# NVIDIA-Merlin/NVTabular

Hardware: AMD Instinct MI355X
Metric: rows/sec + GB/s (Criteo Categorify+FillMissing+Normalize fit+transform, HBM-resident) (higher is better)
Workload: dtype int32 keys -> int64 labels; fp64 moments/normalize; 1 GPU; synthetic Criteo-day0: 26 int32 categorical (Criteo-1TB cardinalities, Zipf) + 13 int32 continuous, nulls as Arrow bitmaps; Categorify + FillMissing + Normalize, fit + transform; rows_per_gpu=45000000, algorithmic_bytes_per_row=624, tie_break=value (count desc, value asc), artifacts=deferred (no parquet I/O inside the timed region)

## Files before the change

### nvtabular_amd/csrc/nvt_sort.hip

```cpp
#include <type_traits>

#include <cstdlib>

#include "nvt_common.hpp"
#include "nvt_internal.hpp"
#include "nvt_prof.hpp"
#include "nvt_scan.hpp"
#include "nvt_sort_tile.hpp"

namespace nvt {

template <typename K>
__device__ __forceinline__ unsigned sort_digit(K key, int64_t cnt, int pass) {
  constexpr int KB = (int)sizeof(K);
  if (pass < KB) {
    using U = typename std::make_unsigned<K>::type;
    U u = (U)key ^ ((U)1 << (8 * KB - 1));
    return (unsigned)((u >> (8 * pass)) & 0xFF);
  }
  uint64_t inv = ~(uint64_t)cnt;
  return (unsigned)((inv >> (8 * (pass - KB))) & 0xFF);
}

constexpr int kSmallMax = 8192;
constexpr int kSmallBS = 1024;

template <typename K>
__device__ __forceinline__ bool vocab_before(int64_t ca, K ka, int64_t cb, K kb) {
  return ca > cb || (ca == cb && ka < kb);
}

template <typename K>
__global__ __launch_bounds__(kSmallBS) void sort_small_kernel(K *keys, int64_t *counts, unsigned n) {
  __shared__ K sk[kSmallMax];
  __shared__ int64_t sc[kSmallMax];
  unsigned m = 1;
  while (m < n) m <<= 1;
  for (unsigned i = threadIdx.x; i < m; i += kSmallBS) {
    if (i < n) {
      sk[i] = keys[i];
      sc[i] = counts[i];
    } else {
      sk[i] = std::numeric_limits<K>::max();
      sc[i] = INT64_MIN;
    }
  }
  __syncthreads();
  for (unsigned size = 2; size <= m; size <<= 1) {
    for (unsigned stride = size >> 1; stride > 0; stride >>= 1) {
      for (unsigned t = threadIdx.x; t < m / 2; t += kSmallBS) {
        unsigned lo = 2 * t - (t & (stride - 1));
        unsigned hi = lo + stride;
        bool up = (lo & size) == 0;
        K ka = sk[lo], kb = sk[hi];
        int64_t ca = sc[lo], cb = sc[hi];
        bool swap = up ? vocab_before<K>(cb, kb, ca, ka) : vocab_before<K>(ca, ka, cb, kb);
        if (swap) {
          sk[lo] = kb;
          sk[hi] = ka;
          sc[lo] = cb;
          sc[hi] = ca;
        }
      }
      __syncthreads();
    }
  }
  for (unsigned i = threadIdx.x; i < n; i += kSmallBS) {
    keys[i] = sk[i];
    counts[i] = sc[i];
  }
}

constexpr int kRows = 8;
constexpr int kTileSort = kBlock * kRows;

template <typename K>
__global__ __launch_bounds__(kBlock) void sort_pass_hist_kernel(const K *__restrict__ keys,
                                                                const int64_t *__restrict__ cnts,
                                                                uint64_t n,
                                                                unsigned long long *pass_hist) {
  constexpr int NP = (int)sizeof(K) + 8;
  __shared__ unsigned h[NP * 256];
  for (int i = threadIdx.x; i < NP * 256; i += kBlock) h[i] = 0;
  __syncthreads();
  const uint64_t stride = (uint64_t)gridDim.x * kBlock;
  for (uint64_t i = (uint64_t)blockIdx.x * kBlock + threadIdx.x; i < n; i += stride) {
    K k = keys[i];
    int64_t c = cnts[i];
#pragma unroll
    for (int p = 0; p < NP; ++p) atomicAdd(&h[p * 256 + sort_digit<K>(k, c, p)], 1u);
  }
  __syncthreads();
  for (int i = threadIdx.x; i < NP * 256; i += kBlock)
    if (h[i]) atomicAdd(&pass_hist[i], (unsigned long long)h[i]);
}

__device__ __forceinline__ uint64_t tile_elem(uint64_t tile, unsigned w, unsigned r, unsigned l) {
  return tile * kTileSort + (uint64_t)w * (kRows * kWave) + (uint64_t)r * kWave + l;
}

template <typename K>
__global__ __launch_bounds__(kBlock) void sort_tile_hist_kernel(const K *__restrict__ keys,
                                                                const int64_t *__restrict__ cnts,
                                                                uint64_t n, int pass,
                                                                unsigned *tile_hist,
                                                                uint64_t ntiles) {
  constexpr int KB = (int)sizeof(K);
  __shared__ unsigned h[256];
  h[threadIdx.x] = 0;
  __syncthreads();
  const unsigned w = threadIdx.x / kWave, l = lane_id();
#pragma unroll
  for (int r = 0; r < kRows; ++r) {
    uint64_t i = tile_elem(blockIdx.x, w, r, l);
    if (i < n) {
      unsigned d = pass < KB ? sort_digit<K>(keys[i], 0, pass) : sort_digit<K>((K)0, cnts[i], pass);
      atomicAdd(&h[d], 1u);
    }
  }
  __syncthreads();
  tile_hist[(uint64_t)threadIdx.x * ntiles + blockIdx.x] = h[threadIdx.x];
}

template <typename K>
__global__ __launch_bounds__(kBlock) void sort_scatter_kernel(
    const K *__restrict__ keys, const int64_t *__restrict__ cnts, uint64_t n, int pass,
    const unsigned *__restrict__ tile_off, uint64_t ntiles, K *out_keys, int64_t *out_cnts) {
  __shared__ unsigned wcnt[kBlock / kWave][256];
  const unsigned w = threadIdx.x / kWave, l = lane_id();
  for (int i = threadIdx.x; i < (kBlock / kWave) * 256; i += kBlock) (&wcnt[0][0])[i] = 0;
  __syncthreads();
  K k[kRows];
  int64_t c[kRows];
  unsigned dig[kRows], local[kRows];
  bool act[kRows];
#pragma unroll
  for (int r = 0; r < kRows; ++r) {
    uint64_t i = tile_elem(blockIdx.x, w, r, l);
    act[r] = i < n;
    k[r] = act[r] ? keys[i] : (K)0;
    c[r] = act[r] ? cnts[i] : 0;
    dig[r] = sort_digit<K>(k[r], c[r], pass);
  }
#pragma unroll
  for (int r = 0; r < kRows; ++r) {
    unsigned long long peers = match_digit(dig[r], act[r]);
    unsigned rank = __popcll(peers & ((1ull << l) - 1ull));
    unsigned before = act[r] ? wcnt[w][dig[r]] : 0;
    __builtin_amdgcn_wave_barrier();
    if (act[r] && rank == 0) wcnt[w][dig[r]] = before + (unsigned)__popcll(peers);
    __builtin_amdgcn_wave_barrier();
    local[r] = before + rank;
  }
  __syncthreads();
  {
    const unsigned d = threadIdx.x;
    unsigned run = tile_off[(uint64_t)d * ntiles + blockIdx.x];
#pragma unroll
    for (int q = 0; q < kBlock / kWave; ++q) {
      unsigned t = wcnt[q][d];
      wcnt[q][d] = run;
      run += t;
    }
  }
  __syncthreads();
#pragma unroll
  for (int r = 0; r < kRows; ++r) {
    if (act[r]) {
      unsigned dst = wcnt[w][dig[r]] + local[r];
      out_keys[dst] = k[r];
      out_cnts[dst] = c[r];
    }
  }
}


template <bool FIRST>
__global__ __launch_bounds__(kS2BS) void sort2_hist_kernel(const uint64_t *__restrict__ comp,
                                                           const int32_t *__restrict__ keys,
                                                           const int64_t *__restrict__ cnts,
                                                           uint64_t n, int shift,
                                                           unsigned *tile_hist, uint64_t ntiles) {
  __shared__ unsigned h[256];
  h[threadIdx.x] = 0;
  __syncthreads();
  const uint64_t base = (uint64_t)blockIdx.x * kS2Tile;
#pragma unroll 4
  for (int r = 0; r < kS2Rows; ++r) {
    const uint64_t i = base + (uint64_t)r * kS2BS + threadIdx.x;
    const bool act = i < n;
    uint64_t c = 0;
    if (act) c = FIRST ? comp_make(keys[i], cnts[i]) : comp[i];
    const unsigned d = (unsigned)(c >> shift) & 0xFF;
    if (shift < 32) {
      if (act) atomicAdd(&h[d], 1u);
    } else {
      const unsigned long long peers = match_digit(d, act);
      if (act && (peers & ((1ull << lane_id()) - 1ull)) == 0)
        atomicAdd(&h[d], (unsigned)__popcll(peers));
    }
  }
  __syncthreads();
  tile_hist[(uint64_t)threadIdx.x * ntiles + blockIdx.x] = h[threadIdx.x];
}

template <bool FIRST, bool LAST>
__global__ __launch_bounds__(kS2BS) void sort2_scatter_kernel(
    const uint64_t *__restrict__ comp, const int32_t *__restrict__ keys,
    const int64_t *__restrict__ cnts, uint64_t n, int shift, const unsigned *__restrict__ tile_off,
    const unsigned long long *__restrict__ chunk_base, uint64_t ntiles, uint64_t *out_comp,
    int32_t *out_keys, int64_t *out_cnts) {
  constexpr int NW = kS2BS / kWave;
  __shared__ unsigned wcnt[NW][256];
  __shared__ unsigned goff[256];
  __shared__ unsigned wtot[NW];
  __shared__ uint64_t stage[kS2Tile];
  const unsigned w = threadIdx.x / kWave, l = lane_id();
#pragma unroll
  for (int q = 0; q < NW; ++q) wcnt[q][threadIdx.x] = 0;
  __syncthreads();
  uint64_t c[kS2Rows];
  unsigned short local[kS2Rows];
#pragma unroll
  for (int r = 0; r < kS2Rows; ++r) {
    const uint64_t i = s2_elem(blockIdx.x, w, r, l);
    c[r] = ~0ull;
    if (i < n) c[r] = FIRST ? comp_make(keys[i], cnts[i]) : comp[i];
  }
  const uint64_t tile_base = (uint64_t)blockIdx.x * kS2Tile;
#pragma unroll
  for (int r = 0; r < kS2Rows; ++r) {
    const bool act = s2_elem(blockIdx.x, w, r, l) < n;
    const unsigned d = (unsigned)(c[r] >> shift) & 0xFF;
    const unsigned long long peers = match_digit(d, act);
    const unsigned rank = __popcll(peers & ((1ull << l) - 1ull));
    const unsigned before = act ? wcnt[w][d] : 0;
    __builtin_amdgcn_wave_barrier();
    if (act && rank == 0) wcnt[w][d] = before + (unsigned)__popcll(peers);
    __builtin_amdgcn_wave_barrier();
    local[r] = (unsigned short)(before + rank);
  }
  __syncthreads();
  {
    const unsigned d = threadIdx.x;
    unsigned t[NW], tot = 0;
#pragma unroll
    for (int q = 0; q < NW; ++q) {
      t[q] = wcnt[q][d];
      tot += t[q];
    }
    unsigned inc = tot;
#pragma unroll
    for (int off = 1; off < 64; off <<= 1) {
      unsigned o = __shfl_up(inc, off, 64);
      if (l >= (unsigned)off) inc += o;
    }
    if (l == 63) wtot[w] = inc;
    __syncthreads();
    unsigned wbase = 0;
    for (unsigned q = 0; q < w; ++q) wbase += wtot[q];
    const unsigned dstart = wbase + inc - tot;
    unsigned run = dstart;
#pragma unroll
    for (int q = 0; q < NW; ++q) {
      wcnt[q][d] = run;
      run += t[q];
    }
    goff[d] = scan_lookup(tile_off, chunk_base, (uint64_t)d * ntiles + blockIdx.x) - dstart;
  }
  __syncthreads();
#pragma unroll
  for (int r = 0; r < kS2Rows; ++r) {
    if (s2_elem(blockIdx.x, w, r, l) < n) {
      const unsigned d = (unsigned)(c[r] >> shift) & 0xFF;
      stage[wcnt[w][d] + local[r]] = c[r];
    }
  }
  __syncthreads();
  const unsigned tile_n = (unsigned)(n - tile_base < (uint64_t)kS2Tile ? n - tile_base : kS2Tile);
#pragma unroll 4
  for (int j = 0; j < kS2Rows; ++j) {
    const unsigned idx = j * kS2BS + threadIdx.x;
    if (idx < tile_n) {
      const uint64_t v = stage[idx];
      const unsigned d = (unsigned)(v >> shift) & 0xFF;
      const unsigned dst = goff[d] + idx;
      if (LAST) {
        out_keys[dst] = comp_key(v);
        out_cnts[dst] = comp_cnt(v);
      } else {
        out_comp[dst] = v;
      }
    }
  }
}

constexpr int kOsMaxPass = 8;
constexpr int kOsHistBlocks = 1024;

__global__ __launch_bounds__(kS2BS) void os_hist_kernel(const int32_t *__restrict__ keys,
                                                        const int64_t *__restrict__ cnts,
                                                        uint64_t n, int npass,
                                                        unsigned *__restrict__ block_hist) {
  __shared__ unsigned h[kOsMaxPass * 256];
  for (int i = threadIdx.x; i < npass * 256; i += kS2BS) h[i] = 0;
  __syncthreads();
  const unsigned l = lane_id();
  unsigned c255[kOsMaxPass];
#pragma unroll
  for (int p = 0; p < kOsMaxPass; ++p) c255[p] = 0;
  const uint64_t stride = (uint64_t)gridDim.x * kS2BS;
  const uint64_t iters = (n + stride - 1) / stride;
  for (uint64_t it = 0; it < iters; ++it) {
    const uint64_t i = it * stride + (uint64_t)blockIdx.x * kS2BS + threadIdx.x;
    const bool act = i < n;
    const uint64_t c = act ? comp_make(keys[i], cnts[i]) : 0ull;
#pragma unroll
    for (int p = 0; p < 4; ++p)
      if (act) atomicAdd(&h[p * 256 + ((unsigned)(c >> (8 * p)) & 0xFF)], 1u);
    if (npass > 4) {
      const unsigned d = (unsigned)(c >> 32) & 0xFF;
      const unsigned long long peers = match_digit(d, act);
      if (act && (peers & ((1ull << l) - 1ull)) == 0)
        atomicAdd(&h[4 * 256 + d], (unsigned)__popcll(peers));
    }
#pragma unroll
    for (int p = 5; p < kOsMaxPass; ++p) {
      if (p < npass && act) {
        const unsigned d = (unsigned)(c >> (8 * p)) & 0xFF;
        if (d == 0xFF)
          ++c255[p];
        else
          atomicAdd(&h[p * 256 + d], 1u);
      }
    }
  }
#pragma unroll
  for (int p = 5; p < kOsMaxPass; ++p) {
    if (p < npass) {
      unsigned v = c255[p];
#pragma unroll
      for (int off = 32; off > 0; off >>= 1) v += __shfl_down(v, off, 64);
      if (l == 0 && v) atomicAdd(&h[p * 256 + 0xFF], v);
    }
  }
  __syncthreads();
  for (int i = threadIdx.x; i < npass * 256; i += kS2BS)
    block_hist[(uint64_t)blockIdx.x * (kOsMaxPass * 256) + i] = h[i];
}

__global__ __launch_bounds__(256) void os_base_kernel(const unsigned *__restrict__ block_hist,
                                                      int nblocks, unsigned *__restrict__ base) {
  __shared__ unsigned wtot[4];
  const int p = blockIdx.x, d = threadIdx.x;
  unsigned tot = 0;
#pragma unroll 8
  for (int b = 0; b < nblocks; ++b) tot += block_hist[(uint64_t)b * (kOsMaxPass * 256) + p * 256 + d];
  unsigned inc = tot;
#pragma unroll
  for (int off = 1; off < 64; off <<= 1) {
    unsigned o = __shfl_up(inc, off, 64);
    if (lane_id() >= (unsigned)off) inc += o;
  }
  const unsigned w = threadIdx.x / kWave;
  if (lane_id() == 63) wtot[w] = inc;
  __syncthreads();
  unsigned wb = 0;
  for (unsigned q = 0; q < w; ++q) wb += wtot[q];
  base[p * 256 + d] = wb + inc - tot;
}

template <bool LAST, typename LOAD>
__device__ __forceinline__ void os_scatter_body(
    LOAD load, uint64_t n, int shift, const unsigned *__restrict__ base,
    unsigned *status, unsigned *ticket, uint64_t *out_comp, int32_t *out_keys, int64_t *out_cnts) {
  constexpr int NW = kS2BS / kWave;
  __shared__ unsigned wcnt[NW][256];
  __shared__ unsigned goff[256];
  __shared__ unsigned wtot[NW];
  __shared__ unsigned s_tile;
  __shared__ uint64_t stage[kS2Tile];
  const unsigned w = threadIdx.x / kWave, l = lane_id();
  if (threadIdx.x == 0) s_tile = atomicAdd(ticket, 1u);
#pragma unroll
  for (int q = 0; q < NW; ++q) wcnt[q][threadIdx.x] = 0;
  __syncthreads();
  const unsigned tile = s_tile;
  uint64_t c[kS2Rows];
  unsigned short local[kS2Rows];
#pragma unroll
  for (int r = 0; r < kS2Rows; ++r) {
    const uint64_t i = s2_elem(tile, w, r, l);
    c[r] = ~0ull;
    if (i < n) c[r] = load(i);
  }
  const uint64_t tile_base = (uint64_t)tile * kS2Tile;
#pragma unroll
  for (int r = 0; r < kS2Rows; ++r) {
    const bool act = s2_elem(tile, w, r, l) < n;
    const unsigned d = (unsigned)(c[r] >> shift) & 0xFF;
    const unsigned long long peers = match_digit(d, act);
    const unsigned rank = __popcll(peers & ((1ull << l) - 1ull));
    const unsigned before = act ? wcnt[w][d] : 0;
    __builtin_amdgcn_wave_barrier();
    if (act && rank == 0) wcnt[w][d] = before + (unsigned)__popcll(peers);
    __builtin_amdgcn_wave_barrier();
    local[r] = (unsigned short)(before + rank);
  }
  __syncthreads();
  {
    const unsigned d = threadIdx.x;
    unsigned t[NW], tot = 0;
#pragma unroll
    for (int q = 0; q < NW; ++q) {
      t[q] = wcnt[q][d];
      tot += t[q];
    }
    unsigned *my = status + (uint64_t)tile * 256 + d;
    __hip_atomic_store(my, (tile == 0 ? kOsPrefix : kOsAgg) | tot, __ATOMIC_RELAXED,
                       __HIP_MEMORY_SCOPE_AGENT);
    unsigned inc = tot;
#pragma unroll
    for (int off = 1; off < 64; off <<= 1) {
      unsigned o = __shfl_up(inc, off, 64);
      if (l >= (unsigned)off) inc += o;
    }
    if (l == 63) wtot[w] = inc;
    __syncthreads();
    unsigned wbase = 0;
    for (unsigned q = 0; q < w; ++q) wbase += wtot[q];
    const unsigned dstart = wbase + inc - tot;
    unsigned run = dstart;
#pragma unroll
    for (int q = 0; q < NW; ++q) {
      wcnt[q][d] = run;
      run += t[q];
    }
    unsigned excl = 0;
    if (tile > 0) {
      unsigned tb = tile - 1;
      while (true) {
        const unsigned v = __hip_atomic_load(status + (uint64_t)tb * 256 + d, __ATOMIC_RELAXED,
                                             __HIP_MEMORY_SCOPE_AGENT);
        const unsigned f = v >> 30;
        if (f == 0) {
          __builtin_amdgcn_s_sleep(1);
          continue;
        }
        excl += v & kOsMask;
        if (f == 2) break;
        --tb;
      }
      __hip_atomic_store(my, kOsPrefix | (excl + tot), __ATOMIC_RELAXED, __HIP_MEMORY_SCOPE_AGENT);
    }
    goff[d] = base[d] + excl - dstart;
  }
  __syncthreads();
#pragma unroll
  for (int r = 0; r < kS2Rows; ++r) {
    if (s2_elem(tile, w, r, l) < n) {
      const unsigned d = (unsigned)(c[r] >> shift) & 0xFF;
      stage[wcnt[w][d] + local[r]] = c[r];
    }
  }
  __syncthreads();
  const unsigned tile_n = (unsigned)(n - tile_base < (uint64_t)kS2Tile ? n - tile_base : kS2Tile);
#pragma unroll 4
  for (int j = 0; j < kS2Rows; ++j) {
    const unsigned idx = j * kS2BS + threadIdx.x;
    if (idx < tile_n) {
      const uint64_t v = stage[idx];
      const unsigned d = (unsigned)(v >> shift) & 0xFF;
      const unsigned dst = goff[d] + idx;
      if (LAST) {
        out_keys[dst] = comp_key(v);
        out_cnts[dst] = comp_cnt(v);
      } else {
        out_comp[dst] = v;
      }
    }
  }
}

template <bool FIRST, bool LAST>
__global__ __launch_bounds__(kS2BS) void os_scatter_kernel(
    const uint64_t *__restrict__ comp, const int32_t *__restrict__ keys,
    const int64_t *__restrict__ cnts, uint64_t n, int shift, const unsigned *__restrict__ base,
    unsigned *status, unsigned *ticket, uint64_t *out_comp, int32_t *out_keys, int64_t *out_cnts) {
  os_scatter_body<LAST>([=](uint64_t i) -> uint64_t { return FIRST ? comp_make(keys[i], cnts[i]) : comp[i]; },
                        n, shift, base, status, ticket, out_comp, out_keys, out_cnts);
}

template <typename K>
struct PackedKeyWord {
  const K *keys;
  const uint8_t *fold;
  int64_t bias;
  int rb;
  __device__ __forceinline__ uint64_t operator()(uint64_t i) const {
    const uint64_t img = (uint32_t)((uint64_t)(int64_t)keys[i] - (uint64_t)bias);
    const uint64_t f = fold ? (uint64_t)fold[i] : 0ull;
    return (img << 32) | (f << rb) | i;
  }
};
template <typename K>
__global__ __launch_bounds__(kS2BS) void os_scatter_pack_kernel(
    PackedKeyWord<K> src, uint64_t n, int shift, const unsigned *__restrict__ base, unsigned *status,
    unsigned *ticket, uint64_t *out_comp) {
  os_scatter_body<false>(src, n, shift, base, status, ticket, out_comp, nullptr, nullptr);
}

inline uint64_t os_tmp_bytes(uint64_t n) {
  const uint64_t ntiles = (n + kS2Tile - 1) / kS2Tile;
  return 2 * n * 8 + (uint64_t)kOsHistBlocks * kOsMaxPass * 256 * 4 + kOsMaxPass * 256 * 4 +
         (uint64_t)kOsMaxPass * ntiles * 256 * 4 + kOsMaxPass * 4 + 256;
}

inline int vocab_sort_onesweep(int32_t *keys, int64_t *counts, uint64_t n, int64_t max_count,
                               void *tmp, hipStream_t stream) {
  const uint64_t ntiles = (n + kS2Tile - 1) / kS2Tile;
  char *p = reinterpret_cast<char *>(tmp);
  uint64_t *bufs[2];
  bufs[0] = reinterpret_cast<uint64_t *>(p);
  p += n * 8;
  bufs[1] = reinterpret_cast<uint64_t *>(p);
  p += n * 8;
  unsigned *block_hist = reinterpret_cast<unsigned *>(p);
  p += (uint64_t)kOsHistBlocks * kOsMaxPass * 256 * 4;
  unsigned *base = reinterpret_cast<unsigned *>(p);
  p += kOsMaxPass * 256 * 4;
  unsigned *status = reinterpret_cast<unsigned *>(p);
  int count_bytes = 0;
  for (uint64_t m = (uint64_t)max_count; m; m >>= 8) ++count_bytes;
  const int npass = 4 + count_bytes;
  const uint64_t status_words = (uint64_t)npass * ntiles * 256;
  unsigned *tickets = status + status_words;
  NVT_CHECK_HIP(hipMemsetAsync(status, 0, (status_words + kOsMaxPass) * 4, stream));
  const unsigned hb = (unsigned)(ntiles < (uint64_t)kOsHistBlocks ? ntiles : kOsHistBlocks);
  os_hist_kernel<<<hb, kS2BS, 0, stream>>>(keys, counts, n, npass, block_hist);
  NVT_CHECK_LAUNCH();
  os_base_kernel<<<npass, 256, 0, stream>>>(block_hist, (int)hb, base);
  NVT_CHECK_LAUNCH();
  const uint64_t *src = nullptr;
  int flip = 0;
  for (int pass = 0; pass < npass; ++pass) {
    const int shift = 8 * pass;
    const bool first = pass == 0, last = pass == npass - 1;
    unsigned *st = status + (uint64_t)pass * ntiles * 256;
    uint64_t *dst = bufs[flip];
    if (first)
      os_scatter_kernel<true, false><<<(unsigned)ntiles, kS2BS, 0, stream>>>(
          nullptr, keys, counts, n, shift, base + pass * 256, st, tickets + pass, dst, nullptr,
          nullptr);
    else if (last)
      os_scatter_kernel<false, true><<<(unsigned)ntiles, kS2BS, 0, stream>>>(
          src, nullptr, nullptr, n, shift, base + pass * 256, st, tickets + pass, nullptr, keys,
          counts);
    else
      os_scatter_kernel<false, false><<<(unsigned)ntiles, kS2BS, 0, stream>>>(
          src, nullptr, nullptr, n, shift, base + pass * 256, st, tickets + pass, dst, nullptr,
          nullptr);
    NVT_CHECK_LAUNCH();
    src = dst;
    flip ^= 1;
  }
  return NVT_OK;
}

template <typename LOAD>
__device__ __forceinline__ void os_hist_words_body(LOAD load, uint64_t n, int bit_lo, int npass,
                                                   unsigned *__restrict__ block_hist) {
  __shared__ unsigned h[kOsMaxPass * 256];
  for (int i = threadIdx.x; i < npass * 256; i += kS2BS) h[i] = 0;
  __syncthreads();
  const unsigned l = lane_id();
  const uint64_t stride = (uint64_t)gridDim.x * kS2BS;
  const uint64_t iters = (n + stride - 1) / stride;
  constexpr int U = 4;
  for (uint64_t it = 0; it < iters; it += U) {
    uint64_t cw[U];
    bool av[U];
#pragma unroll
    for (int u = 0; u < U; ++u) {
      const uint64_t i = (it + u) * stride + (uint64_t)blockIdx.x * kS2BS + threadIdx.x;
      av[u] = (it + u) < iters && i < n;
      cw[u] = av[u] ? load(i) >> bit_lo : 0ull;
    }
#pragma unroll
    for (int u = 0; u < U; ++u) {
      const bool act = av[u];
      const uint64_t c = cw[u];
#pragma unroll
      for (int p = 0; p < kOsMaxPass; ++p) {
        if (p < npass) {
          const unsigned d = (unsigned)(c >> (8 * p)) & 0xFF;
          const unsigned long long am = __ballot(act);
          const unsigned d0 = __builtin_amdgcn_readfirstlane(d);
          if (am == ~0ull && __ballot(d == d0) == ~0ull) {
            if (l == 0) atomicAdd(&h[p * 256 + d0], 64u);
          } else if (act) {
            atomicAdd(&h[p * 256 + d], 1u);
          }
        }
      }
    }
  }
  __syncthreads();
  for (int i = threadIdx.x; i < npass * 256; i += kS2BS)
    block_hist[(uint64_t)blockIdx.x * (kOsMaxPass * 256) + i] = h[i];
}

__global__ __launch_bounds__(kS2BS) void os_hist_words_kernel(const uint64_t *__restrict__ w,
                                                              uint64_t n, int bit_lo, int npass,
                                                              unsigned *__restrict__ block_hist) {
  os_hist_words_body([=](uint64_t i) -> uint64_t { return w[i]; }, n, bit_lo, npass, block_hist);
}
template <typename K>
__global__ __launch_bounds__(kS2BS) void os_hist_pack_kernel(PackedKeyWord<K> src, uint64_t n, int bit_lo,
                                                             int npass, unsigned *__restrict__ block_hist) {
  os_hist_words_body(src, n, bit_lo, npass, block_hist);
}

uint64_t sort_words_tmp_bytes(uint64_t n) { return os_tmp_bytes(n); }

static int sort_words_impl(uint64_t *data, const void *keys, int key_dtype, int64_t key_bias,
                           const uint8_t *fold, int rb, uint64_t n, int bit_lo, int bit_hi, void *tmp,
                           uint64_t **result, hipStream_t stream) {
  NVT_CHECK_ARG(n < (1ull << 30), "at most 2^30-1 words");
  const int npass = (bit_hi - bit_lo + 7) / 8;
  NVT_CHECK_ARG(npass >= 1 && npass <= kOsMaxPass, "bit range too wide");
  const uint64_t ntiles = (n + kS2Tile - 1) / kS2Tile;
  char *p = reinterpret_cast<char *>(tmp);
  uint64_t *bufs[2];
  bufs[0] = reinterpret_cast<uint64_t *>(p);
  p += n * 8;
  bufs[1] = reinterpret_cast<uint64_t *>(p);
  p += n * 8;
  unsigned *block_hist = reinterpret_cast<unsigned *>(p);
  p += (uint64_t)kOsHistBlocks * kOsMaxPass * 256 * 4;
  unsigned *base = reinterpret_cast<unsigned *>(p);
  p += kOsMaxPass * 256 * 4;
  unsigned *status = reinterpret_cast<unsigned *>(p);
  const uint64_t status_words = (uint64_t)npass * ntiles * 256;
  unsigned *tickets = status + status_words;
  NVT_CHECK_HIP(hipMemsetAsync(status, 0, (status_words + kOsMaxPass) * 4, stream));
  const unsigned hb = (unsigned)(ntiles < (uint64_t)kOsHistBlocks ? ntiles : kOsHistBlocks);
  const PackedKeyWord<int32_t> s32{reinterpret_cast<const int32_t *>(keys), fold, key_bias, rb};
  const PackedKeyWord<int64_t> s64{reinterpret_cast<const int64_t *>(keys), fold, key_bias, rb};
  if (!keys)
    os_hist_words_kernel<<<hb, kS2BS, 0, stream>>>(data, n, bit_lo, npass, block_hist);
  else if (key_dtype == NVT_I32)
    os_hist_pack_kernel<int32_t><<<hb, kS2BS, 0, stream>>>(s32, n, bit_lo, npass, block_hist);
  else
    os_hist_pack_kernel<int64_t><<<hb, kS2BS, 0, stream>>>(s64, n, bit_lo, npass, block_hist);
  NVT_CHECK_LAUNCH();
  os_base_kernel<<<npass, 256, 0, stream>>>(block_hist, (int)hb, base);
  NVT_CHECK_LAUNCH();
  const uint64_t *src = data;
  int flip = 0;
  for (int pass = 0; pass < npass; ++pass) {
    uint64_t *dst = bufs[flip];
    unsigned *st = status + (uint64_t)pass * ntiles * 256;
    if (pass == 0 && keys && key_dtype == NVT_I32)
      os_scatter_pack_kernel<int32_t><<<(unsigned)ntiles, kS2BS, 0, stream>>>(
          s32, n, bit_lo, base, st, tickets, dst);
    else if (pass == 0 && keys)
      os_scatter_pack_kernel<int64_t><<<(unsigned)ntiles, kS2BS, 0, stream>>>(
          s64, n, bit_lo, base, st, tickets, dst);
    else
      os_scatter_kernel<false, false><<<(unsigned)ntiles, kS2BS, 0, stream>>>(
          src, nullptr, nullptr, n, bit_lo + 8 * pass, base + pass * 256, st, tickets + pass, dst,
          nullptr, nullptr);
    NVT_CHECK_LAUNCH();
    src = dst;
    flip ^= 1;
  }
  *result = const_cast<uint64_t *>(src);
  return NVT_OK;
}

int sort_words_bits(uint64_t *data, uint64_t n, int bit_lo, int bit_hi, void *tmp, uint64_t **result,
                    hipStream_t stream) {
  *result = data;
  if (n <= 1 || bit_hi <= bit_lo) return NVT_OK;
  return sort_words_impl(data, nullptr, 0, 0, nullptr, 0, n, bit_lo, bit_hi, tmp, result, stream);
}

int sort_packed_keys(const void *keys, int key_dtype, int64_t key_bias, const uint8_t *fold, int rb,
                     uint64_t n, void *tmp, uint64_t **result, hipStream_t stream) {
  NVT_CHECK_ARG(keys && n >= 1 && rb >= 24 && rb <= 32, "keys / rows / row bits");
  return sort_words_impl(nullptr, keys, key_dtype, key_bias, fold, rb, n, rb, 64, tmp, result, stream);
}

constexpr int kSmallPackedMax = 16384;
struct SmallCol {
  int32_t *keys;
  int64_t *counts;
  unsigned n;
};
constexpr int kSmallBatch = 64;
struct SmallBatch {
  SmallCol c[kSmallBatch];
};
__global__ __launch_bounds__(kSmallBS) void sort_small_packed_many_kernel(SmallBatch b) {
  __shared__ uint64_t sv[kSmallPackedMax];
  const SmallCol col = b.c[blockIdx.x];
  const unsigned n = col.n;
  unsigned m = 1;
  while (m < n) m <<= 1;
  for (unsigned i = threadIdx.x; i < m; i += kSmallBS)
    sv[i] = i < n ? comp_make(col.keys[i], col.counts[i]) : ~0ull;
  __syncthreads();
  for (unsigned size = 2; size <= m; size <<= 1) {
    for (unsigned stride = size >> 1; stride > 0; stride >>= 1) {
      for (unsigned t = threadIdx.x; t < m / 2; t += kSmallBS) {
        const unsigned lo = 2 * t - (t & (stride - 1));
        const unsigned hi = lo + stride;
        const bool up = (lo & size) == 0;
        const uint64_t a = sv[lo], c = sv[hi];
        if (up ? (c < a) : (a < c)) {
          sv[lo] = c;
          sv[hi] = a;
        }
      }
      __syncthreads();
    }
  }
  for (unsigned i = threadIdx.x; i < n; i += kSmallBS) {
    const uint64_t v = sv[i];
    col.keys[i] = comp_key(v);
    col.counts[i] = comp_cnt(v);
  }
}

inline uint64_t sort2_tmp_bytes(uint64_t n) {
  const uint64_t ntiles = (n + kS2Tile - 1) / kS2Tile, hist_len = 256 * ntiles;
  return 2 * n * 8 + pad16(hist_len * 4) + scan_chunks(hist_len) * 8 + 64;
}

inline int vocab_sort_packed(int32_t *keys, int64_t *counts, uint64_t n, int64_t max_count,
                             void *tmp, hipStream_t stream) {
  const uint64_t ntiles = (n + kS2Tile - 1) / kS2Tile, hist_len = 256 * ntiles;
  char *p = reinterpret_cast<char *>(tmp);
  uint64_t *bufs[2];
  bufs[0] = reinterpret_cast<uint64_t *>(p);
  p += n * 8;
  bufs[1] = reinterpret_cast<uint64_t *>(p);
  p += n * 8;
  unsigned *tile_hist = reinterpret_cast<unsigned *>(p);
  p += pad16(hist_len * 4);
  unsigned long long *chunk_tot = reinterpret_cast<unsigned long long *>(p);
  int count_bytes = 0;
  for (uint64_t m = (uint64_t)max_count; m; m >>= 8) ++count_bytes;
  const int npass = 4 + count_bytes;
  const uint64_t *src = nullptr;
  int flip = 0;
  for (int pass = 0; pass < npass; ++pass) {
    const int shift = 8 * pass;
    const bool first = pass == 0, last = pass == npass - 1;
    if (first)
      sort2_hist_kernel<true><<<(unsigned)ntiles, kS2BS, 0, stream>>>(nullptr, keys, counts, n,
                                                                       shift, tile_hist, ntiles);
    else
      sort2_hist_kernel<false><<<(unsigned)ntiles, kS2BS, 0, stream>>>(src, nullptr, nullptr, n,
                                                                        shift, tile_hist, ntiles);
    NVT_CHECK_LAUNCH();
    const unsigned long long *cbase = nullptr;
    {
      int rc = exclusive_scan_u32_deferred(tile_hist, hist_len, chunk_tot, &cbase, stream);
      if (rc) return rc;
    }
    uint64_t *dst = bufs[flip];
    if (first)
      sort2_scatter_kernel<true, false><<<(unsigned)ntiles, kS2BS, 0, stream>>>(
          nullptr, keys, counts, n, shift, tile_hist, cbase, ntiles, dst, nullptr, nullptr);
    else if (last)
      sort2_scatter_kernel<false, true><<<(unsigned)ntiles, kS2BS, 0, stream>>>(
          src, nullptr, nullptr, n, shift, tile_hist, cbase, ntiles, nullptr, keys, counts);
    else
      sort2_scatter_kernel<false, false><<<(unsigned)ntiles, kS2BS, 0, stream>>>(
          src, nullptr, nullptr, n, shift, tile_hist, cbase, ntiles, dst, nullptr, nullptr);
    NVT_CHECK_LAUNCH();
    src = dst;
    flip ^= 1;
  }
  return NVT_OK;
}

template <typename K>
int vocab_sort(K *keys, int64_t *counts, uint64_t n, int64_t max_count, void *tmp,
               hipStream_t stream) {
  constexpr int NP = (int)sizeof(K) + 8;
  if (n <= 1) return NVT_OK;
  NVT_CHECK_ARG(n < (1ull << 32), "at most 2^32-1 vocabulary entries");
  if (n <= kSmallMax) {
    sort_small_kernel<K><<<1, kSmallBS, 0, stream>>>(keys, counts, (unsigned)n);
    NVT_CHECK_LAUNCH();
    return NVT_OK;
  }
  if constexpr (sizeof(K) == 4) {
    if (max_count > 0 && max_count < (1ll << 32) && n < (1ull << 30))
      return vocab_sort_onesweep(keys, counts, n, max_count, tmp, stream);
    if (max_count > 0 && max_count < (1ll << 32) && n < (1ull << 31))
      return vocab_sort_packed(keys, counts, n, max_count, tmp, stream);
  }
  const uint64_t ntiles = (n + kTileSort - 1) / kTileSort;
  char *p = reinterpret_cast<char *>(tmp);
  int64_t *counts2 = reinterpret_cast<int64_t *>(p);
  p += n * sizeof(int64_t);
  K *keys2 = reinterpret_cast<K *>(p);
  p += pad16(n * sizeof(K));
  unsigned *tile_hist = reinterpret_cast<unsigned *>(p);
  const uint64_t hist_len = 256 * ntiles;
  p += pad16(hist_len * sizeof(unsigned));
  const uint64_t nchunks = (hist_len + kScanChunk - 1) / kScanChunk;
  unsigned long long *chunk_tot = reinterpret_cast<unsigned long long *>(p);
  p += nchunks * sizeof(unsigned long long);
  unsigned long long *pass_hist = reinterpret_cast<unsigned long long *>(p);

  bool run_pass[NP];
  if (max_count > 0) {
    constexpr int KB = (int)sizeof(K);
    int count_bytes = 0;
    for (uint64_t m = (uint64_t)max_count; m; m >>= 8) ++count_bytes;
    for (int p = 0; p < NP; ++p) run_pass[p] = p < KB || (p - KB) < count_bytes;
  } else {
    NVT_CHECK_HIP(hipMemsetAsync(pass_hist, 0, NP * 256 * sizeof(unsigned long long), stream));
    sort_pass_hist_kernel<K><<<stream_grid(n, kBlock * 8, 4), kBlock, 0, stream>>>(keys, counts, n,
                                                                                     pass_hist);
    NVT_CHECK_LAUNCH();
    unsigned long long host_hist[NP * 256];
    NVT_CHECK_HIP(hipMemcpyAsync(host_hist, pass_hist, sizeof(host_hist), hipMemcpyDeviceToHost,
                                 stream));
    NVT_CHECK_HIP(hipStreamSynchronize(stream));
    for (int p = 0; p < NP; ++p) {
      run_pass[p] = true;
      for (int d = 0; d < 256; ++d)
        if (host_hist[p * 256 + d] == n) run_pass[p] = false;
    }
  }

  K *src_k = keys, *dst_k = keys2;
  int64_t *src_c = counts, *dst_c = counts2;
  for (int pass = 0; pass < NP; ++pass) {
    if (!run_pass[pass]) continue;
    sort_tile_hist_kernel<K><<<(unsigned)ntiles, kBlock, 0, stream>>>(src_k, src_c, n, pass,
                                                                      tile_hist, ntiles);
    NVT_CHECK_LAUNCH();
    {
      int rc = exclusive_scan_u32(tile_hist, hist_len, chunk_tot, stream);
      if (rc) return rc;
    }
    sort_scatter_kernel<K><<<(unsigned)ntiles, kBlock, 0, stream>>>(src_k, src_c, n, pass,
                                                                    tile_hist, ntiles, dst_k, dst_c);
    NVT_CHECK_LAUNCH();
    K *tk = src_k;
    src_k = dst_k;
    dst_k = tk;
    int64_t *tc = src_c;
    src_c = dst_c;
    dst_c = tc;
  }
  if (src_k != keys) {
    NVT_CHECK_HIP(hipMemcpyAsync(keys, src_k, n * sizeof(K), hipMemcpyDeviceToDevice, stream));
    NVT_CHECK_HIP(
        hipMemcpyAsync(counts, src_c, n * sizeof(int64_t), hipMemcpyDeviceToDevice, stream));
  }
  return NVT_OK;
}

int vocab_sort_any(int key_bytes, void *keys, int64_t *counts, uint64_t n, int64_t max_count,
                   void *tmp, hipStream_t s) {
  NVT_PROF("vocab_sort", 0, s);
  if (key_bytes == 4) return vocab_sort<int32_t>((int32_t *)keys, counts, n, max_count, tmp, s);
  return vocab_sort<int64_t>((int64_t *)keys, counts, n, max_count, tmp, s);
}

bool vocab_sort_small_eligible(int key_bytes, uint64_t n, int64_t max_count) {
  return key_bytes == 4 && n >= 2 && n <= (uint64_t)kSmallPackedMax && max_count > 0 &&
         max_count < (1ll << 32);
}

int vocab_sort_small_batch(const SmallSortDesc *cols, int ncols, hipStream_t s) {
  for (int c0 = 0; c0 < ncols; c0 += kSmallBatch) {
    const int nc = ncols - c0 < kSmallBatch ? ncols - c0 : kSmallBatch;
    SmallBatch b;
    memset(&b, 0, sizeof(b));
    for (int i = 0; i < nc; ++i) {
      b.c[i].keys = cols[c0 + i].keys;
      b.c[i].counts = cols[c0 + i].counts;
      b.c[i].n = cols[c0 + i].n;
    }
    NVT_PROF("vocab_sort_small", 0, s);
    sort_small_packed_many_kernel<<<nc, kSmallBS, 0, s>>>(b);
    NVT_CHECK_LAUNCH();
  }
  return NVT_OK;
}

}

using namespace nvt;

extern "C" {

int nvt_vocab_sort_tmp_bytes(int key_bytes, uint64_t n, uint64_t *bytes) {
  NVT_CHECK_ARG(bytes && (key_bytes == 4 || key_bytes == 8), "key_bytes must be 4 or 8");
  const uint64_t ntiles = (n + kTileSort - 1) / kTileSort;
  const uint64_t hist_len = 256 * ntiles;
  const uint64_t nchunks = (hist_len + kScanChunk - 1) / kScanChunk;
  *bytes = n * 8 + pad16(n * key_bytes) + pad16(hist_len * 4) + nchunks * 8 +
           (uint64_t)(key_bytes + 8) * 256 * 8 + 64;
  if (key_bytes == 4 && sort2_tmp_bytes(n) > *bytes) *bytes = sort2_tmp_bytes(n);
  if (key_bytes == 4 && os_tmp_bytes(n) > *bytes) *bytes = os_tmp_bytes(n);
  return NVT_OK;
}
int nvt_vocab_sort_i32(int32_t *keys, int64_t *counts, uint64_t n, int64_t max_count, void *tmp,
                       void *stream) {
  NVT_CHECK_ARG(n <= 1 || (keys && counts && tmp), "null pointer");
  return vocab_sort_any(4, keys, counts, n, max_count, tmp, (hipStream_t)stream);
}
int nvt_vocab_sort_i64(int64_t *keys, int64_t *counts, uint64_t n, int64_t max_count, void *tmp,
                       void *stream) {
  NVT_CHECK_ARG(n <= 1 || (keys && counts && tmp), "null pointer");
  return vocab_sort_any(8, keys, counts, n, max_count, tmp, (hipStream_t)stream);
}

}
```

Before: 4.933 billion rows/s.

## Register-blocked bitonic sort for mid-size vocabularies and route single-column sorts to it

For vocabularies between 8192 and 16384 entries, the small packed sort now keeps 16 elements per thread in registers. It runs up to four bitonic stages locally before writing back to padded shared memory, which cuts barrier count and LDS traffic. The padding (one slot per 16) avoids bank conflicts. vocab_sort also sends eligible int32 single-column sorts to this packed kernel ahead of the generic small sort. The index and mirror logic is intricate and risks subtle correctness bugs, and it may raise register pressure.

```diff
diff --git a/nvtabular_amd/csrc/nvt_sort.hip b/nvtabular_amd/csrc/nvt_sort.hip
--- a/nvtabular_amd/csrc/nvt_sort.hip
+++ b/nvtabular_amd/csrc/nvt_sort.hip
@@ -693,6 +693,10 @@
 }
 
 constexpr int kSmallPackedMax = 16384;
+constexpr unsigned kSmallBlockedMin = 8192;
+constexpr int kSmallRegLog2 = 4, kSmallReg = 1 << kSmallRegLog2;
+constexpr int kSmallSlots = kSmallPackedMax + kSmallPackedMax / 16;
+static_assert(kSmallBS * kSmallReg == kSmallPackedMax, "a thread per 16 words at the largest size");
 struct SmallCol {
   int32_t *keys;
   int64_t *counts;
@@ -702,34 +706,122 @@
 struct SmallBatch {
   SmallCol c[kSmallBatch];
 };
+__device__ __forceinline__ unsigned small_slot(unsigned i) { return i + (i >> 4); }
+
+__device__ __forceinline__ void small_cx(uint64_t &a, uint64_t &c) {
+  const uint64_t x = a, y = c;
+  const bool sw = y < x;
+  a = sw ? y : x;
+  c = sw ? x : y;
+}
+template <int RB>
+__device__ __forceinline__ void small_stage(uint64_t (&v)[kSmallReg], unsigned live) {
+#pragma unroll
+  for (int r = 0; r < kSmallReg; ++r) {
+    if (r & (1 << RB)) continue;
+    if ((unsigned)(r | (1 << RB)) < live) small_cx(v[r], v[r | (1 << RB)]);
+  }
+}
+template <int TOP>
+__device__ __forceinline__ void small_mirror(uint64_t (&v)[kSmallReg], unsigned live) {
+#pragma unroll
+  for (int r = 0; r < kSmallReg; ++r) {
+    if (r & (1 << TOP)) continue;
+    if ((unsigned)(r ^ ((2 << TOP) - 1)) < live) small_cx(v[r], v[r ^ ((2 << TOP) - 1)]);
+  }
+}
+
 __global__ __launch_bounds__(kSmallBS) void sort_small_packed_many_kernel(SmallBatch b) {
-  __shared__ uint64_t sv[kSmallPackedMax];
+  __shared__ uint64_t sv[kSmallSlots];
   const SmallCol col = b.c[blockIdx.x];
   const unsigned n = col.n;
-  unsigned m = 1;
-  while (m < n) m <<= 1;
+  if (n <= kSmallBlockedMin) {
+    unsigned m = 1;
+    while (m < n) m <<= 1;
+    for (unsigned i = threadIdx.x; i < m; i += kSmallBS)
+      sv[i] = i < n ? comp_make(col.keys[i], col.counts[i]) : ~0ull;
+    __syncthreads();
+    for (unsigned size = 2; size <= m; size <<= 1) {
+      for (unsigned stride = size >> 1; stride > 0; stride >>= 1) {
+        for (unsigned t = threadIdx.x; t < m / 2; t += kSmallBS) {
+          const unsigned lo = 2 * t - (t & (stride - 1));
+          const unsigned hi = lo + stride;
+          const bool up = (lo & size) == 0;
+          const uint64_t a = sv[lo], c = sv[hi];
+          if (up ? (c < a) : (a < c)) {
+            sv[lo] = c;
+            sv[hi] = a;
+          }
+        }
+        __syncthreads();
+      }
+    }
+    for (unsigned i = threadIdx.x; i < n; i += kSmallBS) {
+      const uint64_t v = sv[i];
+      col.keys[i] = comp_key(v);
+      col.counts[i] = comp_cnt(v);
+    }
+    return;
+  }
+  constexpr unsigned lg = 14, m = 1u << lg;
+  static_assert(m == (unsigned)kSmallPackedMax && kSmallBlockedMin * 2 == kSmallPackedMax, "one padded size");
   for (unsigned i = threadIdx.x; i < m; i += kSmallBS)
-    sv[i] = i < n ? comp_make(col.keys[i], col.counts[i]) : ~0ull;
-  __syncthreads();
-  for (unsigned size = 2; size <= m; size <<= 1) {
-    for (unsigned stride = size >> 1; stride > 0; stride >>= 1) {
-      for (unsigned t = threadIdx.x; t < m / 2; t += kSmallBS) {
-        const unsigned lo = 2 * t - (t & (stride - 1));
-        const unsigned hi = lo + stride;
-        const bool up = (lo & size) == 0;
-        const uint64_t a = sv[lo], c = sv[hi];
-        if (up ? (c < a) : (a < c)) {
-          sv[lo] = c;
-          sv[hi] = a;
+    sv[small_slot(i)] = i < n ? comp_make(col.keys[i], col.counts[i]) : ~0ull;
+  __syncthreads();
+  const unsigned t = threadIdx.x;
+  uint64_t v[kSmallReg];
+  unsigned base = 0, fmask = 0, live = 0;
+  int held = -1;
+  auto slot_of = [&](int r) {
+    return small_slot((base | ((unsigned)r << held)) ^ ((r & (kSmallReg / 2)) ? fmask : 0u));
+  };
+  auto put_back = [&]() {
+#pragma unroll
+    for (int r = 0; r < kSmallReg; ++r)
+      if ((unsigned)r < live) sv[slot_of(r)] = v[r];
+  };
+  for (unsigned k = 1; k <= lg; ++k) {
+    for (int j = (int)k - 1; j >= 0;) {
+      const int lo = j >= kSmallRegLog2 - 1 ? j - (kSmallRegLog2 - 1) : 0;
+      const bool first = j == (int)k - 1;
+      const unsigned lowmask = (1u << lo) - 1u, fm = first ? lowmask : 0u;
+      if (lo != held || fm != fmask) {
+        if (held >= 0) {
+          put_back();
+          __syncthreads();
         }
+        held = lo;
+        fmask = fm;
+        base = (t & lowmask) | ((t >> lo) << (lo + kSmallRegLog2));
+        const unsigned floor_i = lo < 6 ? (t & ~(unsigned)(kWave - 1)) << kSmallRegLog2 : base & ~lowmask;
+        const unsigned step_log2 = lo < 6 ? 0u : (unsigned)lo;
+        unsigned cnt = n > floor_i ? (n - floor_i + ((1u << step_log2) - 1u)) >> step_log2 : 0u;
+        cnt = lo < 6 ? (cnt ? (unsigned)kSmallReg : 0u) : (cnt < (unsigned)kSmallReg ? cnt : (unsigned)kSmallReg);
+        live = (unsigned)__builtin_amdgcn_readfirstlane((int)cnt);
+#pragma unroll
+        for (int r = 0; r < kSmallReg; ++r) v[r] = (unsigned)r < live ? sv[slot_of(r)] : ~0ull;
       }
-      __syncthreads();
-    }
-  }
+      const int top = j - lo;
+      if (first) {
+        if (top == 3) small_mirror<3>(v, live);
+        else if (top == 2) small_mirror<2>(v, live);
+        else if (top == 1) small_mirror<1>(v, live);
+        else small_mirror<0>(v, live);
+      }
+      const int ptop = first ? top - 1 : top;
+      if (ptop >= 3) small_stage<3>(v, live);
+      if (ptop >= 2) small_stage<2>(v, live);
+      if (ptop >= 1) small_stage<1>(v, live);
+      if (ptop >= 0) small_stage<0>(v, live);
+      j = lo - 1;
+    }
+  }
+  put_back();
+  __syncthreads();
   for (unsigned i = threadIdx.x; i < n; i += kSmallBS) {
-    const uint64_t v = sv[i];
-    col.keys[i] = comp_key(v);
-    col.counts[i] = comp_cnt(v);
+    const uint64_t w = sv[small_slot(i)];
+    col.keys[i] = comp_key(w);
+    col.counts[i] = comp_cnt(w);
   }
 }
 
@@ -793,6 +885,18 @@
   constexpr int NP = (int)sizeof(K) + 8;
   if (n <= 1) return NVT_OK;
   NVT_CHECK_ARG(n < (1ull << 32), "at most 2^32-1 vocabulary entries");
+  if constexpr (sizeof(K) == 4) {
+    if (vocab_sort_small_eligible(4, n, max_count)) {
+      SmallBatch b;
+      memset(&b, 0, sizeof(b));
+      b.c[0].keys = keys;
+      b.c[0].counts = counts;
+      b.c[0].n = (unsigned)n;
+      sort_small_packed_many_kernel<<<1, kSmallBS, 0, stream>>>(b);
+      NVT_CHECK_LAUNCH();
+      return NVT_OK;
+    }
+  }
   if (n <= kSmallMax) {
     sort_small_kernel<K><<<1, kSmallBS, 0, stream>>>(keys, counts, (unsigned)n);
     NVT_CHECK_LAUNCH();
```

Measured after the change: 4.843 billion rows/s. 0.982x the previous value.
